# BiaPyX/BiaPy

Measured on AMD Instinct MI355X. Metric: voxels/sec 3D ResUNet 128^3 patch (train: fwd+bwd+AdamW; sub-records: infer, sliding), higher is better.
Workload: dtype f16 forward/activations + bf16 gradients (MFMA f16 / bf16, fp32 accumulate)

## Files before the change

### biapy_amd/_lib.py

```python
from __future__ import annotations

import ctypes as C
import os
from typing import Optional

import torch

_HERE = os.path.dirname(os.path.abspath(__file__))
LIB_PATH = os.environ.get("BPX_LIB_PATH") or os.path.join(_HERE, "libbiapy_amd.so")

F32, BF16, F16, U8, MIX16 = 0, 1, 2, 3, 4
U16 = 5
I32 = 6
ACT = {"none": 0, "linear": 0, "elu": 1, "relu": 2, "silu": 3, "leaky_relu": 4, "gelu": 5, "tanh": 6, "sigmoid": 7, "softplus": 8}
PK_K3, PK_K3_T, PK_K1, PK_DENSE, PK_DENSE_T, PK_CT, PK_CT_T, PK_CT4, PK_CT4_T = range(9)


class AxisGrid(C.Structure):
    _fields_ = [("n", C.c_int32), ("step", C.c_int32), ("last", C.c_int32), ("patch", C.c_int32), ("limit", C.c_int32)]


class Tensor(C.Structure):
    _fields_ = [("ptr", C.c_void_p), ("ld", C.c_int32), ("C", C.c_int32), ("cs", C.c_int64)]

# ... 95 lines not shown
    "bpx_conv3d_wgrad": ([_i, _i, _i, _i, _i, Tensor, _vp, _i, Tensor, _i, _vp, _vp, _vp, _i64, _vp], _i),
    "bpx_conv3d_wgrad_db2": ([_i, _i, _i, _i, _i, Tensor, _vp, _i, Tensor, _i, _vp, _vp, _vp, _vp, _i64, _vp], _i),
    "bpx_conv3d_wgrad_workspace": ([_i, _i, _i, _i, _i, _i, _i], _i64),
    "bpx_conv3d_bwd_fused_supported": ([_i, _i, _i, _i, _i, _i, _i], _i),
    "bpx_conv3d_bwd_fused_stats_tiles": ([_i, _i, _i, _i, _i, _i], _i),
    "bpx_conv3d_bwd_fused_workspace": ([_i, _i, _i, _i, _i, _i], _i64),
    "bpx_conv3d_bwd_fused": ([_i, _i, _i, _i, _i, Tensor, _vp, Tensor, _vp, _i, Tensor, _vp, _vp, _vp, _vp, _vp, _i64, _vp], _i),
    "bpx_debug_set_bwd_fused": ([_i], _i),
    "bpx_debug_set_bwd_rs": ([_i], _i),
    "bpx_debug_set_conv_kg": ([_i], _i),
    "bpx_debug_set_tile_order": ([_i], _i),
    "bpx_debug_set_wgrad_cap": ([_i], _i),
    "bpx_debug_set_wgrad_k1": ([_i], _i),
    "bpx_debug_set_pw_stream": ([_i], _i),
    "bpx_debug_set_convt_k1": ([_i], _i),
    "bpx_debug_set_c1_persist": ([_i], _i),
    "bpx_convT3d_k2s2_wgrad_workspace": ([_i, _i, _i, _i, _i, _i, _i], _i64),
    "bpx_conv1x1_fwd": ([_i, _i, _i64, Tensor, _vp, _vp, Tensor, Tensor, _vp, Tensor, Tensor, _vp], _i),
    "bpx_conv1x1_fwd_split_wgrad_workspace": ([_i, _i, _i64, _i], _i64),
    "bpx_conv1x1_fwd_split_wgrad_query": ([_i, _i, _i64, Tensor, Tensor, Tensor, _vp, Tensor, Tensor], _i64),
    "bpx_conv1x1_fwd_split_wgrad": ([_i, _i, _i64, Tensor, _vp, Tensor, Tensor, _vp, Tensor, Tensor, _vp, _vp, _i64, _vp], _i),
    "bpx_conv1x1_fwd_split": ([_i, _i, _i64, Tensor, _vp, _vp, Tensor, Tensor, _vp, Tensor, Tensor, Tensor, _vp], _i),
    "bpx_convT3d_k2s2_fwd": ([_i, _i, _i, _i, _i, _i, Tensor, _vp, _vp, Tensor, _vp, _vp], _i),
    "bpx_convT3d_stats_tiles": ([_i, _i, _i, _i], _i),
    "bpx_convT3d_k2s2_dgrad": ([_i, _i, _i, _i, _i, _i, Tensor, _vp, Tensor, _vp], _i),
    "bpx_convT3d_k2s2_wgrad": ([_i, _i, _i, _i, _i, _i, Tensor, Tensor, _vp, _vp, _vp, _i64, _vp], _i),
    "bpx_convT3d_k2s2_bwd": ([_i, _i, _i, _i, _i, _i, Tensor, Tensor, _vp, Tensor, _vp, _vp, _vp, _i64, _vp], _i),
    "bpx_debug_set_convt_bwd": ([_i], _i),
    "bpx_debug_convt_bwd_launches": ([], _i),
    "bpx_norm_finalize": ([_vp, _i, _i, _i, _i64, _vp, _vp, _f, _i, _vp, _i, _i, _vp], _i),
# ... 239 lines not shown
```

### biapy_amd/csrc/pointwise.hip

```cpp
#include <type_traits>

#include <cstdlib>

#include "bpx_common.h"

#ifndef BPX_PW_MS_CT
#define BPX_PW_MS_CT 2
#endif
#ifndef BPX_CONVT_OCC
#define BPX_CONVT_OCC 2
#endif
#ifndef BPX_CONVT_PD
#define BPX_CONVT_PD 2
#endif

namespace {

enum { PW_CONV1 = 0, PW_CONVT = 1, PW_CONVTD = 2 };

template <typename T> __device__ __forceinline__ void load4(const T* p, float* f);
template <> __device__ __forceinline__ void load4<uint16_t>(const uint16_t* p, float* f) {
  u32x2_t v = *reinterpret_cast<const u32x2_t*>(p);
  f[0] = bf16lo(v[0]); f[1] = bf16hi(v[0]); f[2] = bf16lo(v[1]); f[3] = bf16hi(v[1]);
}
template <> __device__ __forceinline__ void load4<float>(const float* p, float* f) {
  f32x4_t v = *reinterpret_cast<const f32x4_t*>(p);
  f[0] = v[0]; f[1] = v[1]; f[2] = v[2]; f[3] = v[3];
}

template <typename T, int NQ> __device__ __forceinline__ void loadq(const T* p, float (*f)[4]);
template <typename T, int NQ> __device__ __forceinline__ void storeq(T* p, const float (*f)[4]);
template <> __device__ __forceinline__ void loadq<float, 1>(const float* p, float (*f)[4]) { load4<float>(p, f[0]); }
template <> __device__ __forceinline__ void loadq<float, 2>(const float* p, float (*f)[4]) { load4<float>(p, f[0]); load4<float>(p + 4, f[1]); }
template <> __device__ __forceinline__ void loadq<float, 3>(const float* p, float (*f)[4]) { load4<float>(p, f[0]); load4<float>(p + 4, f[1]); load4<float>(p + 8, f[2]); }
template <> __device__ __forceinline__ void loadq<float, 4>(const float* p, float (*f)[4]) { load4<float>(p, f[0]); load4<float>(p + 4, f[1]); load4<float>(p + 8, f[2]); load4<float>(p + 12, f[3]); }
__device__ __forceinline__ void load8_bf16(const uint16_t* p, float* f0, float* f1) {
  u32x4_t v = *reinterpret_cast<const u32x4_t*>(p);
  f0[0] = bf16lo(v[0]); f0[1] = bf16hi(v[0]); f0[2] = bf16lo(v[1]); f0[3] = bf16hi(v[1]);
  f1[0] = bf16lo(v[2]); f1[1] = bf16hi(v[2]); f1[2] = bf16lo(v[3]); f1[3] = bf16hi(v[3]);
}
template <> __device__ __forceinline__ void loadq<uint16_t, 1>(const uint16_t* p, float (*f)[4]) { load4<uint16_t>(p, f[0]); }
template <> __device__ __forceinline__ void loadq<uint16_t, 2>(const uint16_t* p, float (*f)[4]) { load8_bf16(p, f[0], f[1]); }
template <> __device__ __forceinline__ void loadq<uint16_t, 3>(const uint16_t* p, float (*f)[4]) { load8_bf16(p, f[0], f[1]); load4<uint16_t>(p + 8, f[2]); }
template <> __device__ __forceinline__ void loadq<uint16_t, 4>(const uint16_t* p, float (*f)[4]) { load8_bf16(p, f[0], f[1]); load8_bf16(p + 8, f[2], f[3]); }
template <int NQ> __device__ __forceinline__ void storeq_f32(float* p, const float (*f)[4]) {
#pragma unroll
  for (int q = 0; q < NQ; ++q) *reinterpret_cast<f32x4_t*>(p + 4 * q) = f32x4_t{f[q][0], f[q][1], f[q][2], f[q][3]};
}
template <> __device__ __forceinline__ void storeq<float, 1>(float* p, const float (*f)[4]) { storeq_f32<1>(p, f); }
template <> __device__ __forceinline__ void storeq<float, 2>(float* p, const float (*f)[4]) { storeq_f32<2>(p, f); }
template <> __device__ __forceinline__ void storeq<float, 3>(float* p, const float (*f)[4]) { storeq_f32<3>(p, f); }
template <> __device__ __forceinline__ void storeq<float, 4>(float* p, const float (*f)[4]) { storeq_f32<4>(p, f); }
__device__ __forceinline__ void store4_bf16(uint16_t* p, const float* f) {
  *reinterpret_cast<u32x2_t*>(p) = u32x2_t{pack_bf16x2(f[0], f[1]), pack_bf16x2(f[2], f[3])};
}
__device__ __forceinline__ void store8_bf16(uint16_t* p, const float* f0, const float* f1) {
  *reinterpret_cast<u32x4_t*>(p) = u32x4_t{pack_bf16x2(f0[0], f0[1]), pack_bf16x2(f0[2], f0[3]), pack_bf16x2(f1[0], f1[1]), pack_bf16x2(f1[2], f1[3])};
}
template <> __device__ __forceinline__ void storeq<uint16_t, 1>(uint16_t* p, const float (*f)[4]) { store4_bf16(p, f[0]); }
template <> __device__ __forceinline__ void storeq<uint16_t, 2>(uint16_t* p, const float (*f)[4]) { store8_bf16(p, f[0], f[1]); }
template <> __device__ __forceinline__ void storeq<uint16_t, 3>(uint16_t* p, const float (*f)[4]) { store8_bf16(p, f[0], f[1]); store4_bf16(p + 8, f[2]); }
template <> __device__ __forceinline__ void storeq<uint16_t, 4>(uint16_t* p, const float (*f)[4]) { store8_bf16(p, f[0], f[1]); store8_bf16(p + 8, f[2], f[3]); }

template <> __device__ __forceinline__ void load4<f16_t>(const f16_t* p, float* f) {
  u32x2_t v = *reinterpret_cast<const u32x2_t*>(p);
  f[0] = lo16<f16_t>(v[0]); f[1] = hi16<f16_t>(v[0]); f[2] = lo16<f16_t>(v[1]); f[3] = hi16<f16_t>(v[1]);
}
__device__ __forceinline__ void load8_f16(const f16_t* p, float* f0, float* f1) {
  u32x4_t v = *reinterpret_cast<const u32x4_t*>(p);
  f0[0] = lo16<f16_t>(v[0]); f0[1] = hi16<f16_t>(v[0]); f0[2] = lo16<f16_t>(v[1]); f0[3] = hi16<f16_t>(v[1]);
  f1[0] = lo16<f16_t>(v[2]); f1[1] = hi16<f16_t>(v[2]); f1[2] = lo16<f16_t>(v[3]); f1[3] = hi16<f16_t>(v[3]);
}
template <> __device__ __forceinline__ void loadq<f16_t, 1>(const f16_t* p, float (*f)[4]) { load4<f16_t>(p, f[0]); }
template <> __device__ __forceinline__ void loadq<f16_t, 2>(const f16_t* p, float (*f)[4]) { load8_f16(p, f[0], f[1]); }
template <> __device__ __forceinline__ void loadq<f16_t, 3>(const f16_t* p, float (*f)[4]) { load8_f16(p, f[0], f[1]); load4<f16_t>(p + 8, f[2]); }
template <> __device__ __forceinline__ void loadq<f16_t, 4>(const f16_t* p, float (*f)[4]) { load8_f16(p, f[0], f[1]); load8_f16(p + 8, f[2], f[3]); }
__device__ __forceinline__ void store4_f16(f16_t* p, const float* f) {
  *reinterpret_cast<u32x2_t*>(p) = u32x2_t{pk16s<f16_t>(f[0], f[1]), pk16s<f16_t>(f[2], f[3])};
}
__device__ __forceinline__ void store8_f16(f16_t* p, const float* f0, const float* f1) {
  *reinterpret_cast<u32x4_t*>(p) = u32x4_t{pk16s<f16_t>(f0[0], f0[1]), pk16s<f16_t>(f0[2], f0[3]), pk16s<f16_t>(f1[0], f1[1]), pk16s<f16_t>(f1[2], f1[3])};
}
template <> __device__ __forceinline__ void storeq<f16_t, 1>(f16_t* p, const float (*f)[4]) { store4_f16(p, f[0]); }
template <> __device__ __forceinline__ void storeq<f16_t, 2>(f16_t* p, const float (*f)[4]) { store8_f16(p, f[0], f[1]); }
template <> __device__ __forceinline__ void storeq<f16_t, 3>(f16_t* p, const float (*f)[4]) { store8_f16(p, f[0], f[1]); store4_f16(p + 8, f[2]); }
template <> __device__ __forceinline__ void storeq<f16_t, 4>(f16_t* p, const float (*f)[4]) { store8_f16(p, f[0], f[1]); store8_f16(p + 8, f[2], f[3]); }

template <typename T, int NQ> __device__ __forceinline__ void loadq_planar(const T* vbase, int c0, int cs, float (*f)[4]) {
  auto at = [&](int c) { return vbase + (size_t)(c >> 4) * cs + (c & 15); };
  if (NQ == 1) loadq<T, 1>(at(c0), f);
  else if (NQ == 2) loadq<T, 2>(at(c0), f);
  else if (NQ == 4) { loadq<T, 2>(at(c0), f); loadq<T, 2>(at(c0 + 8), f + 2); }
  else if (sizeof(T) == 4) { loadq<T, 1>(at(c0), f); loadq<T, 1>(at(c0 + 4), f + 1); loadq<T, 1>(at(c0 + 8), f + 2); }
  else {
    const int b0 = c0 & ~7;
    float a[2][4], b[2][4];
    loadq<T, 2>(at(b0), a);
    loadq<T, 2>(at(b0 + 8), b);
    const bool odd = (c0 & 7) != 0;
#pragma unroll
    for (int r = 0; r < 4; ++r) {
      f[0][r] = odd ? a[1][r] : a[0][r];
      f[1][r] = odd ? b[0][r] : a[1][r];
      f[2][r] = odd ? b[1][r] : b[0][r];
    }
  }
}
template <typename T, int NQ> __device__ __forceinline__ void storeq_planar(T* vbase, int c0, int cs, const float (*f)[4]) {
  auto at = [&](int c) { return vbase + (size_t)(c >> 4) * cs + (c & 15); };
  if (NQ == 1) storeq<T, 1>(at(c0), f);
  else if (NQ == 2) storeq<T, 2>(at(c0), f);
  else if (NQ == 4) { storeq<T, 2>(at(c0), f); storeq<T, 2>(at(c0 + 8), f + 2); }
  else if ((c0 & 7) == 0) { storeq<T, 2>(at(c0), f); storeq<T, 1>(at(c0 + 8), f + 2); }
  else { storeq<T, 1>(at(c0), f); storeq<T, 2>(at(c0 + 4), f + 1); }
}

struct PwParams {
  int N, D, H, W;
  int sz;
  int64_t vps;
  const void* x; int x_ld; int K;
  int Csub;
  const void* wp; const float* bias;
  void* y; int y_ld; int Ncols;
  void* y2; int y2_ld; int ysplit;
  const void* g; int g_ld; const void* t; int t_ld; const bpx_nbwd_coef* coef;
  int t_cs, y_cs;
  const void* addend; int addend_ld;
  float* part; int mblocks;
  uint32_t y_bytes;
  int mgroups;
};

template <typename T, int MS, int NS, int MODE, bool PL, typename TT = T, bool K1STEP = false>
__global__ void __launch_bounds__(256) pw_kernel(const PwParams p) {
  using Tr = ElemTraits<T>;
  constexpr int KPL = Tr::KPL;
  const int tid = threadIdx.x, lane = tid & 63, wave = tid >> 6;
  const int j = lane & 15, g = lane >> 4;
  const int nbk = p.Ncols / (16 * NS);
  const unsigned bid = blockIdx.x;
  const int nb = bid % nbk;
  const int grp = (bid / nbk) % p.mgroups;
  const int n = bid / (nbk * p.mgroups);
  const int col_base = nb * 16 * NS;
  constexpr bool PERM = MODE == PW_CONVT && PL && NS == 4;
  const int ppb = PERM ? p.Csub / 32 : 1;
// ... 554 lines not shown
        }
      }
    __syncthreads();
    if (tid < NS * 16 * 2) {
      const int c = tid >> 1, k = tid & 1;
      const float a = red[(0 * NS * 16 + c) * 2 + k] + red[(1 * NS * 16 + c) * 2 + k] + red[(2 * NS * 16 + c) * 2 + k] + red[(3 * NS * 16 + c) * 2 + k];
      const int gg = c >> 4, ns = (c >> 2) & 3;
      const int sub_c = 2 * sp + (gg >> 1);
      const int co = pp * 32 + (ns >> 1) * 16 + (gg & 1) * 8 + (ns & 1) * 4 + (c & 3);
      p.part[((((size_t)n * p.mgroups + grp) * (4 * p.sz) + sub_c) * 2 + k) * p.Csub + co] = a;
    }
  }
}

int g_pw_stream = 1;
int g_convt_k1 = -1;
constexpr int PW_MS = 2;
constexpr int PW_MS_CT = BPX_PW_MS_CT;

inline int convt_groups(int64_t vps) { return (int)std::min<int64_t>(cdiv64(vps, 64 * PW_MS_CT), 64); }

inline int pw_ns(int ncols_per_group) { return (ncols_per_group % 64 == 0) ? 4 : (ncols_per_group % 48 == 0) ? 3 : (ncols_per_group % 32 == 0) ? 2 : 1; }

template <typename T, int MODE, typename TT = T>
int launch_pw(PwParams& p, int ns, hipStream_t s) {
  constexpr int MSK = (MODE == PW_CONVT) ? PW_MS_CT : PW_MS;
  if (p.vps >= (1ll << 31) - 64 * MSK) { bpx_set_error("pointwise kernels: more than 2^31 voxels per sample"); return 1; }
  p.mblocks = (int)cdiv64(p.vps, 64 * MSK);
  p.mgroups = MODE == PW_CONVT ? convt_groups(p.vps) : p.mblocks;
  int nbk = p.Ncols / (16 * ns);
  dim3 grid((unsigned)((int64_t)p.N * p.mgroups * nbk));
  const bool planar = (MODE == PW_CONV1 && p.coef != nullptr && p.t_cs != 16) || (MODE == PW_CONVT && p.y_cs != 16);
  if (MODE == PW_CONVT && planar && ns == 4 && p.Csub % 32 != 0) { bpx_set_error("transposed conv: the 64-column planar form needs Cout % 32 == 0"); return 1; }
  if (MODE != PW_CONVTD && planar) {
    constexpr bool PL = MODE != PW_CONVTD;
    if constexpr (MODE == PW_CONVT && sizeof(T) == 2) {
      const int64_t ovox = (int64_t)p.N * p.vps * 4 * p.sz;
      const int64_t ybytes = ((int64_t)(p.Csub / 16 - 1) * p.y_cs + (ovox - 1) * p.y_ld + 16) * 2;
      static const bool k1_env = getenv("BPX_CONVT_K1") == nullptr || atoi(getenv("BPX_CONVT_K1")) != 0;
      const bool k1 = g_convt_k1 < 0 ? k1_env : g_convt_k1 != 0;
      if (k1 && ns == 4 && p.K * 2 <= 64 && p.W % 16 == 0 && p.vps * p.x_ld * 2 < 0xFFFFFF00ll && ybytes < 0xFFFFFF00ll) {
        p.y_bytes = (uint32_t)ybytes;
        convt_k1_kernel<T><<<grid, 256, 0, s>>>(p);
        return 0;
      }
    }
    if (ns == 4 && MODE == PW_CONVT && sizeof(T) == 2 && p.K * (int)sizeof(T) <= 64) pw_kernel<T, MSK, 4, MODE, PL, TT, MODE == PW_CONVT && sizeof(T) == 2><<<grid, 256, 0, s>>>(p);
    else if (ns == 4) pw_kernel<T, MSK, 4, MODE, PL, TT><<<grid, 256, 0, s>>>(p);
// ... 9 lines not shown
  return 0;
}

int chk(const char* fn, const char* name, const bpx_tensor& t, int es) {
  BPX_CHECK(t.ptr != nullptr, "%s: %s.ptr is null", fn, name);
  BPX_CHECK(t.C % 16 == 0 && t.ld >= (t.cs ? 16 : t.C), "%s: %s needs C %% 16 == 0 and ld >= C (C=%d ld=%d)", fn, name, t.C, t.ld);
  BPX_CHECK(t.cs == 0 || t.cs % 8 == 0, "%s: %s has chunk stride %lld (must be a multiple of 8 elements)", fn, name, (long long)t.cs);
  BPX_CHECK(((uintptr_t)t.ptr % 16) == 0 && ((size_t)t.ld * es) % 16 == 0, "%s: %s must be 16-byte aligned", fn, name);
  return 0;
}

}

extern "C" int bpx_debug_set_pw_stream(int on) { g_pw_stream = on; return 0; }
extern "C" int bpx_debug_set_convt_k1(int on) { g_convt_k1 = on; return 0; }
extern "C" int bpx_convT3d_stats_tiles(int D, int H, int W, int sz) { return convt_groups((int64_t)D * H * W) * 4 * (sz == 1 ? 1 : 2); }

static bool pws_ok(int dtype, int N, int64_t vps, const bpx_tensor& x, bool has_coef, const float* bias_d, const bpx_tensor& g, const bpx_tensor& t,
                   const void* coef_d, const bpx_tensor& addend, const bpx_tensor& y, const bpx_tensor& y2) {
  const int KC = x.C / 16;
  const int TV = KC == 1 ? 128 : 64;
  const int64_t vox = (int64_t)N * vps;
  auto span = [&](const bpx_tensor& q, int chunks) { return (q.cs ? (int64_t)q.cs * (chunks - 1) : 0) * 2 + vox * (int64_t)q.ld * 2; };
  return g_pw_stream && dtype == BPX_BF16 && (KC == 1 || KC == 2) && x.C % 16 == 0 && has_coef && y2.ptr != nullptr && y.C + y2.C == 3 * x.C && y.C % 4 == 0 &&
         g.C == 3 * x.C && t.C == 3 * x.C && bias_d == nullptr && addend.ptr == nullptr && vps % TV == 0 && vox >= 262144 &&
         span(x, 1) < (1ll << 31) && span(g, 1) < (1ll << 31) && span(t, 3 * KC) < (1ll << 31) && (x.ld & 7) == 0 && (g.ld & 7) == 0 && (t.ld & 7) == 0 &&
         (y.ld & 3) == 0 && (y2.ld & 3) == 0 && (((uintptr_t)x.ptr | (uintptr_t)g.ptr | (uintptr_t)t.ptr | (uintptr_t)coef_d) & 15) == 0 &&
         (((uintptr_t)y.ptr | (uintptr_t)y2.ptr) & 7) == 0;
}

// ... 148 lines not shown
```

### include/biapy_amd.h

```cpp
#ifndef BIAPY_AMD_H
#define BIAPY_AMD_H

#include <stdint.h>

#ifdef __cplusplus
extern "C" {
#endif

typedef void* bpx_stream_t;

enum bpx_dtype { BPX_F32 = 0, BPX_BF16 = 1, BPX_F16 = 2, BPX_U8 = 3,
                 BPX_MIX16 = 4,
                 BPX_U16 = 5,
                 BPX_I32 = 6 };
enum bpx_act { BPX_ACT_NONE = 0, BPX_ACT_ELU = 1, BPX_ACT_RELU = 2, BPX_ACT_SILU = 3, BPX_ACT_LEAKY_RELU = 4, BPX_ACT_GELU = 5, BPX_ACT_TANH = 6,
               BPX_ACT_SIGMOID = 7, BPX_ACT_SOFTPLUS = 8, BPX_ACT_LAST = 8 };
enum bpx_pad_mode { BPX_PAD_REFLECT = 0, BPX_PAD_ZEROS = 1 };

int bpx_version(void);
const char* bpx_last_error(void);
int bpx_selftest_layouts(float* out_d , bpx_stream_t stream);
int bpx_debug_set_wgrad_tr(int use_tr);
int bpx_debug_set_conv_stamps(void* stamps_d);
int bpx_debug_set_conv_ws(int on);
int bpx_debug_set_conv_occ(int wg_per_cu);
int bpx_debug_set_conv_zm(int mode);
int bpx_debug_conv_zm_launches(void);
int bpx_debug_conv_zm_occupancy(int nch);
int bpx_debug_set_c1_persist(int wgs);
int bpx_debug_set_convt_k1(int on);
int bpx_debug_set_pw_stream(int on);
int bpx_debug_set_wgrad_k1(int on);
int bpx_debug_set_wgrad_cap(int percent);
int bpx_debug_set_tile_order(int bits);
int bpx_debug_set_tiling_scalar(int on);

typedef struct bpx_axis_grid {
  int32_t n, step, last, patch, limit;
} bpx_axis_grid;

int bpx_crop3d_gather(const void* vol_d, int elem_size, int Z, int Y, int X, int C,
                      int pad_z, int pad_y, int pad_x, int pad_mode,
                      const bpx_axis_grid* grid_zyx ,
                      int64_t c_begin, int64_t c_count, void* out_d, bpx_stream_t stream);

// ... 395 lines not shown
```

Baseline: 1.061 billion.

## Add software-pipelined pointwise GEMM kernel for transposed-conv dgrad path

Adds a separate pointwise kernel variant whose K loop keeps several weight and activation fragment loads in flight in register slots ahead of the MFMA steps. By default it is routed only to the transposed-conv dgrad mode, and only when K is large enough, with a bitmask so other modes can opt in. Shared helpers move into a common header. The intent is to hide global load latency in the K loop; the cost is higher register pressure, which could lower occupancy.

```diff
diff --git a/biapy_amd/_lib.py b/biapy_amd/_lib.py
--- a/biapy_amd/_lib.py
+++ b/biapy_amd/_lib.py
@@ -133,6 +133,7 @@
     "bpx_debug_set_wgrad_k1": ([_i], _i),
     "bpx_debug_set_pw_stream": ([_i], _i),
     "bpx_debug_set_convt_k1": ([_i], _i),
+    "bpx_debug_set_pw_pipeline": ([_i], _i),
     "bpx_debug_set_c1_persist": ([_i], _i),
     "bpx_convT3d_k2s2_wgrad_workspace": ([_i, _i, _i, _i, _i, _i, _i], _i64),
     "bpx_conv1x1_fwd": ([_i, _i, _i64, Tensor, _vp, _vp, Tensor, Tensor, _vp, Tensor, Tensor, _vp], _i),
diff --git a/biapy_amd/csrc/pointwise.hip b/biapy_amd/csrc/pointwise.hip
--- a/biapy_amd/csrc/pointwise.hip
+++ b/biapy_amd/csrc/pointwise.hip
@@ -14,123 +14,10 @@
 #define BPX_CONVT_PD 2
 #endif
 
+#include "pointwise_shared.h"
+
 namespace {
 
-enum { PW_CONV1 = 0, PW_CONVT = 1, PW_CONVTD = 2 };
-
-template <typename T> __device__ __forceinline__ void load4(const T* p, float* f);
-template <> __device__ __forceinline__ void load4<uint16_t>(const uint16_t* p, float* f) {
-  u32x2_t v = *reinterpret_cast<const u32x2_t*>(p);
-  f[0] = bf16lo(v[0]); f[1] = bf16hi(v[0]); f[2] = bf16lo(v[1]); f[3] = bf16hi(v[1]);
-}
-template <> __device__ __forceinline__ void load4<float>(const float* p, float* f) {
-  f32x4_t v = *reinterpret_cast<const f32x4_t*>(p);
-  f[0] = v[0]; f[1] = v[1]; f[2] = v[2]; f[3] = v[3];
-}
-
-template <typename T, int NQ> __device__ __forceinline__ void loadq(const T* p, float (*f)[4]);
-template <typename T, int NQ> __device__ __forceinline__ void storeq(T* p, const float (*f)[4]);
-template <> __device__ __forceinline__ void loadq<float, 1>(const float* p, float (*f)[4]) { load4<float>(p, f[0]); }
-template <> __device__ __forceinline__ void loadq<float, 2>(const float* p, float (*f)[4]) { load4<float>(p, f[0]); load4<float>(p + 4, f[1]); }
-template <> __device__ __forceinline__ void loadq<float, 3>(const float* p, float (*f)[4]) { load4<float>(p, f[0]); load4<float>(p + 4, f[1]); load4<float>(p + 8, f[2]); }
-template <> __device__ __forceinline__ void loadq<float, 4>(const float* p, float (*f)[4]) { load4<float>(p, f[0]); load4<float>(p + 4, f[1]); load4<float>(p + 8, f[2]); load4<float>(p + 12, f[3]); }
-__device__ __forceinline__ void load8_bf16(const uint16_t* p, float* f0, float* f1) {
-  u32x4_t v = *reinterpret_cast<const u32x4_t*>(p);
-  f0[0] = bf16lo(v[0]); f0[1] = bf16hi(v[0]); f0[2] = bf16lo(v[1]); f0[3] = bf16hi(v[1]);
-  f1[0] = bf16lo(v[2]); f1[1] = bf16hi(v[2]); f1[2] = bf16lo(v[3]); f1[3] = bf16hi(v[3]);
-}
-template <> __device__ __forceinline__ void loadq<uint16_t, 1>(const uint16_t* p, float (*f)[4]) { load4<uint16_t>(p, f[0]); }
-template <> __device__ __forceinline__ void loadq<uint16_t, 2>(const uint16_t* p, float (*f)[4]) { load8_bf16(p, f[0], f[1]); }
-template <> __device__ __forceinline__ void loadq<uint16_t, 3>(const uint16_t* p, float (*f)[4]) { load8_bf16(p, f[0], f[1]); load4<uint16_t>(p + 8, f[2]); }
-template <> __device__ __forceinline__ void loadq<uint16_t, 4>(const uint16_t* p, float (*f)[4]) { load8_bf16(p, f[0], f[1]); load8_bf16(p + 8, f[2], f[3]); }
-template <int NQ> __device__ __forceinline__ void storeq_f32(float* p, const float (*f)[4]) {
-#pragma unroll
-  for (int q = 0; q < NQ; ++q) *reinterpret_cast<f32x4_t*>(p + 4 * q) = f32x4_t{f[q][0], f[q][1], f[q][2], f[q][3]};
-}
-template <> __device__ __forceinline__ void storeq<float, 1>(float* p, const float (*f)[4]) { storeq_f32<1>(p, f); }
-template <> __device__ __forceinline__ void storeq<float, 2>(float* p, const float (*f)[4]) { storeq_f32<2>(p, f); }
-template <> __device__ __forceinline__ void storeq<float, 3>(float* p, const float (*f)[4]) { storeq_f32<3>(p, f); }
-template <> __device__ __forceinline__ void storeq<float, 4>(float* p, const float (*f)[4]) { storeq_f32<4>(p, f); }
-__device__ __forceinline__ void store4_bf16(uint16_t* p, const float* f) {
-  *reinterpret_cast<u32x2_t*>(p) = u32x2_t{pack_bf16x2(f[0], f[1]), pack_bf16x2(f[2], f[3])};
-}
-__device__ __forceinline__ void store8_bf16(uint16_t* p, const float* f0, const float* f1) {
-  *reinterpret_cast<u32x4_t*>(p) = u32x4_t{pack_bf16x2(f0[0], f0[1]), pack_bf16x2(f0[2], f0[3]), pack_bf16x2(f1[0], f1[1]), pack_bf16x2(f1[2], f1[3])};
-}
-template <> __device__ __forceinline__ void storeq<uint16_t, 1>(uint16_t* p, const float (*f)[4]) { store4_bf16(p, f[0]); }
-template <> __device__ __forceinline__ void storeq<uint16_t, 2>(uint16_t* p, const float (*f)[4]) { store8_bf16(p, f[0], f[1]); }
-template <> __device__ __forceinline__ void storeq<uint16_t, 3>(uint16_t* p, const float (*f)[4]) { store8_bf16(p, f[0], f[1]); store4_bf16(p + 8, f[2]); }
-template <> __device__ __forceinline__ void storeq<uint16_t, 4>(uint16_t* p, const float (*f)[4]) { store8_bf16(p, f[0], f[1]); store8_bf16(p + 8, f[2], f[3]); }
-
-template <> __device__ __forceinline__ void load4<f16_t>(const f16_t* p, float* f) {
-  u32x2_t v = *reinterpret_cast<const u32x2_t*>(p);
-  f[0] = lo16<f16_t>(v[0]); f[1] = hi16<f16_t>(v[0]); f[2] = lo16<f16_t>(v[1]); f[3] = hi16<f16_t>(v[1]);
-}
-__device__ __forceinline__ void load8_f16(const f16_t* p, float* f0, float* f1) {
-  u32x4_t v = *reinterpret_cast<const u32x4_t*>(p);
-  f0[0] = lo16<f16_t>(v[0]); f0[1] = hi16<f16_t>(v[0]); f0[2] = lo16<f16_t>(v[1]); f0[3] = hi16<f16_t>(v[1]);
-  f1[0] = lo16<f16_t>(v[2]); f1[1] = hi16<f16_t>(v[2]); f1[2] = lo16<f16_t>(v[3]); f1[3] = hi16<f16_t>(v[3]);
-}
-template <> __device__ __forceinline__ void loadq<f16_t, 1>(const f16_t* p, float (*f)[4]) { load4<f16_t>(p, f[0]); }
-template <> __device__ __forceinline__ void loadq<f16_t, 2>(const f16_t* p, float (*f)[4]) { load8_f16(p, f[0], f[1]); }
-template <> __device__ __forceinline__ void loadq<f16_t, 3>(const f16_t* p, float (*f)[4]) { load8_f16(p, f[0], f[1]); load4<f16_t>(p + 8, f[2]); }
-template <> __device__ __forceinline__ void loadq<f16_t, 4>(const f16_t* p, float (*f)[4]) { load8_f16(p, f[0], f[1]); load8_f16(p + 8, f[2], f[3]); }
-__device__ __forceinline__ void store4_f16(f16_t* p, const float* f) {
-  *reinterpret_cast<u32x2_t*>(p) = u32x2_t{pk16s<f16_t>(f[0], f[1]), pk16s<f16_t>(f[2], f[3])};
-}
-__device__ __forceinline__ void store8_f16(f16_t* p, const float* f0, const float* f1) {
-  *reinterpret_cast<u32x4_t*>(p) = u32x4_t{pk16s<f16_t>(f0[0], f0[1]), pk16s<f16_t>(f0[2], f0[3]), pk16s<f16_t>(f1[0], f1[1]), pk16s<f16_t>(f1[2], f1[3])};
-}
-template <> __device__ __forceinline__ void storeq<f16_t, 1>(f16_t* p, const float (*f)[4]) { store4_f16(p, f[0]); }
-template <> __device__ __forceinline__ void storeq<f16_t, 2>(f16_t* p, const float (*f)[4]) { store8_f16(p, f[0], f[1]); }
-template <> __device__ __forceinline__ void storeq<f16_t, 3>(f16_t* p, const float (*f)[4]) { store8_f16(p, f[0], f[1]); store4_f16(p + 8, f[2]); }
-template <> __device__ __forceinline__ void storeq<f16_t, 4>(f16_t* p, const float (*f)[4]) { store8_f16(p, f[0], f[1]); store8_f16(p + 8, f[2], f[3]); }
-
-template <typename T, int NQ> __device__ __forceinline__ void loadq_planar(const T* vbase, int c0, int cs, float (*f)[4]) {
-  auto at = [&](int c) { return vbase + (size_t)(c >> 4) * cs + (c & 15); };
-  if (NQ == 1) loadq<T, 1>(at(c0), f);
-  else if (NQ == 2) loadq<T, 2>(at(c0), f);
-  else if (NQ == 4) { loadq<T, 2>(at(c0), f); loadq<T, 2>(at(c0 + 8), f + 2); }
-  else if (sizeof(T) == 4) { loadq<T, 1>(at(c0), f); loadq<T, 1>(at(c0 + 4), f + 1); loadq<T, 1>(at(c0 + 8), f + 2); }
-  else {
-    const int b0 = c0 & ~7;
-    float a[2][4], b[2][4];
-    loadq<T, 2>(at(b0), a);
-    loadq<T, 2>(at(b0 + 8), b);
-    const bool odd = (c0 & 7) != 0;
-#pragma unroll
-    for (int r = 0; r < 4; ++r) {
-      f[0][r] = odd ? a[1][r] : a[0][r];
-      f[1][r] = odd ? b[0][r] : a[1][r];
-      f[2][r] = odd ? b[1][r] : b[0][r];
-    }
-  }
-}
-template <typename T, int NQ> __device__ __forceinline__ void storeq_planar(T* vbase, int c0, int cs, const float (*f)[4]) {
-  auto at = [&](int c) { return vbase + (size_t)(c >> 4) * cs + (c & 15); };
-  if (NQ == 1) storeq<T, 1>(at(c0), f);
-  else if (NQ == 2) storeq<T, 2>(at(c0), f);
-  else if (NQ == 4) { storeq<T, 2>(at(c0), f); storeq<T, 2>(at(c0 + 8), f + 2); }
-  else if ((c0 & 7) == 0) { storeq<T, 2>(at(c0), f); storeq<T, 1>(at(c0 + 8), f + 2); }
-  else { storeq<T, 1>(at(c0), f); storeq<T, 2>(at(c0 + 4), f + 1); }
-}
-
-struct PwParams {
-  int N, D, H, W;
-  int sz;
-  int64_t vps;
-  const void* x; int x_ld; int K;
-  int Csub;
-  const void* wp; const float* bias;
-  void* y; int y_ld; int Ncols;
-  void* y2; int y2_ld; int ysplit;
-  const void* g; int g_ld; const void* t; int t_ld; const bpx_nbwd_coef* coef;
-  int t_cs, y_cs;
-  const void* addend; int addend_ld;
-  float* part; int mblocks;
-  uint32_t y_bytes;
-  int mgroups;
-};
 
 template <typename T, int MS, int NS, int MODE, bool PL, typename TT = T, bool K1STEP = false>
 __global__ void __launch_bounds__(256) pw_kernel(const PwParams p) {
@@ -715,6 +602,8 @@
 }
 
 int g_pw_stream = 1;
+int g_pw_pipeline = -1;
+constexpr int PW_PIPE_DEFAULT = 8;
 int g_convt_k1 = -1;
 constexpr int PW_MS = 2;
 constexpr int PW_MS_CT = BPX_PW_MS_CT;
@@ -733,6 +622,15 @@
   dim3 grid((unsigned)((int64_t)p.N * p.mgroups * nbk));
   const bool planar = (MODE == PW_CONV1 && p.coef != nullptr && p.t_cs != 16) || (MODE == PW_CONVT && p.y_cs != 16);
   if (MODE == PW_CONVT && planar && ns == 4 && p.Csub % 32 != 0) { bpx_set_error("transposed conv: the 64-column planar form needs Cout % 32 == 0"); return 1; }
+  {
+    static const int pipe_env = getenv("BPX_PW_PIPELINE") == nullptr ? -1 : atoi(getenv("BPX_PW_PIPELINE"));
+    const int pipe_sel = g_pw_pipeline >= 0 ? g_pw_pipeline : pipe_env;
+    const int pipe_mask = pipe_sel < 0 ? PW_PIPE_DEFAULT : pipe_sel == 1 ? 14 : pipe_sel;
+    if (((pipe_mask >> (MODE + 1)) & 1) != 0 && p.K > 4 * ElemTraits<T>::KPL) {
+      const int r = bpx_pw_pipe_launch(MODE, ElemTraits<T>::DT, ElemTraits<TT>::DT, MSK, ns, planar ? 1 : 0, &p, grid.x, s);
+      if (r >= 0) return r;
+    }
+  }
   if (MODE != PW_CONVTD && planar) {
     constexpr bool PL = MODE != PW_CONVTD;
     if constexpr (MODE == PW_CONVT && sizeof(T) == 2) {
@@ -772,6 +670,7 @@
 
 extern "C" int bpx_debug_set_pw_stream(int on) { g_pw_stream = on; return 0; }
 extern "C" int bpx_debug_set_convt_k1(int on) { g_convt_k1 = on; return 0; }
+extern "C" int bpx_debug_set_pw_pipeline(int on) { g_pw_pipeline = on; return 0; }
 extern "C" int bpx_convT3d_stats_tiles(int D, int H, int W, int sz) { return convt_groups((int64_t)D * H * W) * 4 * (sz == 1 ? 1 : 2); }
 
 static bool pws_ok(int dtype, int N, int64_t vps, const bpx_tensor& x, bool has_coef, const float* bias_d, const bpx_tensor& g, const bpx_tensor& t,
diff --git a/biapy_amd/csrc/pointwise_pipe.hip b/biapy_amd/csrc/pointwise_pipe.hip
--- /dev/null
+++ b/biapy_amd/csrc/pointwise_pipe.hip
@@ -0,0 +1,374 @@
+#include "pointwise_shared.h"
+
+#define BPX_CONVT_PD 1
+
+namespace {
+
+template <int I, int N, typename F> __device__ __forceinline__ void pw_static_for(F&& f) {
+  if constexpr (I < N) { f(std::integral_constant<int, I>{}); pw_static_for<I + 1, N>(f); }
+}
+template <typename T, int MS, int NS, int MODE, bool PL, typename TT, bool K1STEP, int PIPE>
+__device__ __forceinline__ void pw_body(const PwParams& p) {
+  using Tr = ElemTraits<T>;
+  constexpr int KPL = Tr::KPL;
+  const int tid = threadIdx.x, lane = tid & 63, wave = tid >> 6;
+  const int j = lane & 15, g = lane >> 4;
+  const int nbk = p.Ncols / (16 * NS);
+  const unsigned bid = blockIdx.x;
+  const int nb = bid % nbk;
+  const int grp = (bid / nbk) % p.mgroups;
+  const int n = bid / (nbk * p.mgroups);
+  const int col_base = nb * 16 * NS;
+  constexpr bool PERM = MODE == PW_CONVT && PL && NS == 4;
+  const int ppb = PERM ? p.Csub / 32 : 1;
+  const int sp = nb / ppb, pp = nb - sp * ppb;
+
+  float s1[NS][4], s2[NS][4];
+#pragma unroll
+  for (int ns = 0; ns < NS; ++ns)
+#pragma unroll
+    for (int r = 0; r < 4; ++r) s1[ns][r] = s2[ns][r] = 0.f;
+  T* __restrict__ yout = reinterpret_cast<T*>(p.y);
+  const T* __restrict__ xin = reinterpret_cast<const T*>(p.x);
+  const T* __restrict__ wp = reinterpret_cast<const T*>(p.wp);
+
+  int mb = grp;
+  constexpr bool PRE = MODE == PW_CONVT && K1STEP;
+  constexpr bool pre = PRE;
+  constexpr int PD = PRE ? BPX_CONVT_PD : 1;
+  u32x4_t af_pre[PD][PRE ? MS : 1], wf_keep[PRE ? NS : 1];
+  auto prefetch = [&](int mbn, auto slot_c) {
+    constexpr int SL = decltype(slot_c)::value;
+#pragma unroll
+    for (int ms = 0; ms < (PRE ? MS : 1); ++ms) {
+      const uint32_t vn = ((uint32_t)mbn * 4u + (uint32_t)wave) * (uint32_t)(MS * 16) + (uint32_t)(ms * 16 + j);
+      af_pre[SL][ms] = u32x4_t{0u, 0u, 0u, 0u};
+      if (g * KPL < p.K && vn < (uint32_t)p.vps) af_pre[SL][ms] = *reinterpret_cast<const u32x4_t*>(xin + ((size_t)n * p.vps + vn) * (size_t)p.x_ld + g * KPL);
+    }
+  };
+  if (pre) {
+    prefetch(mb, std::integral_constant<int, 0>{});
+    if (PD > 1 && mb + p.mgroups < p.mblocks) prefetch(mb + p.mgroups, std::integral_constant<int, (PD > 1 ? 1 : 0)>{});
+    if (PD > 2 && mb + 2 * p.mgroups < p.mblocks) prefetch(mb + 2 * p.mgroups, std::integral_constant<int, (PD > 2 ? 2 : 0)>{});
+    if (PD > 3 && mb + 3 * p.mgroups < p.mblocks) prefetch(mb + 3 * p.mgroups, std::integral_constant<int, (PD > 3 ? 3 : 0)>{});
+#pragma unroll
+    for (int ns = 0; ns < (PRE ? NS : 1); ++ns) {
+      const int gq = j >> 2;
+      const int colw = PERM ? (2 * sp + (gq >> 1)) * p.Csub + pp * 32 + (ns >> 1) * 16 + (gq & 1) * 8 + (ns & 1) * 4 + (j & 3)
+                            : col_base + gq * (4 * NS) + ns * 4 + (j & 3);
+      wf_keep[ns] = *reinterpret_cast<const u32x4_t*>(wp + ((size_t)g * p.Ncols + colw) * KPL);
+    }
+  }
+  const int col0 = col_base + g * 4 * NS;
+  int sub = 0, co0 = col0;
+  if (MODE == PW_CONVT) { sub = col0 / p.Csub; co0 = col0 % p.Csub; }
+  if (PERM) { sub = 2 * sp + (g >> 1); co0 = pp * 32 + (g & 1) * 8; }
+  auto cof = [&](int ns) { return PERM ? co0 + (ns >> 1) * 16 + (ns & 1) * 4 : co0 + ns * 4; };
+  float add[NS][4];
+  auto load_bias = [&]() {
+#pragma unroll
+    for (int ns = 0; ns < NS; ++ns)
+#pragma unroll
+      for (int r = 0; r < 4; ++r) add[ns][r] = p.bias ? p.bias[cof(ns) + r] : 0.f;
+  };
+  if (MODE == PW_CONVT) load_bias();
+  auto one_block = [&](auto slot_c) {
+  constexpr int SL = decltype(slot_c)::value;
+  uint32_t v[MS];
+  bool valid[MS];
+  size_t abase[MS];
+  uint32_t cx[MS], cy[MS], cz[MS];
+#pragma unroll
+  for (int ms = 0; ms < MS; ++ms) {
+    v[ms] = ((uint32_t)mb * 4u + (uint32_t)wave) * (uint32_t)(MS * 16) + (uint32_t)(ms * 16 + j);
+    valid[ms] = v[ms] < (uint32_t)p.vps;
+    const uint32_t vv = valid[ms] ? v[ms] : 0u;
+    if (MODE != PW_CONV1) {
+      const uint32_t row = vv / (uint32_t)p.W;
+      cx[ms] = vv - row * (uint32_t)p.W;
+      cz[ms] = row / (uint32_t)p.H;
+      cy[ms] = row - cz[ms] * (uint32_t)p.H;
+    }
+    if (MODE == PW_CONVTD) {
+      abase[ms] = ((((size_t)n * p.sz * p.D + p.sz * cz[ms]) * 2 * p.H + 2 * cy[ms]) * 2 * p.W + 2 * cx[ms]) * (size_t)p.x_ld;
+    } else {
+      abase[ms] = ((size_t)n * p.vps + vv) * (size_t)p.x_ld;
+    }
+  }
+
+  f32x4_t acc[MS][NS];
+#pragma unroll
+  for (int ms = 0; ms < MS; ++ms)
+#pragma unroll
+    for (int ns = 0; ns < NS; ++ns) acc[ms][ns] = f32x4_t{0.f, 0.f, 0.f, 0.f};
+
+  const int ksteps = (p.K / KPL + 3) / 4;
+  auto plain_loop = [&]() {
+  for (int s = 0; s < ksteps; ++s) {
+    const int k = (4 * s + g) * KPL;
+    const bool kin = k < p.K;
+    u32x4_t wf[NS];
+#pragma unroll
+    for (int ns = 0; ns < NS; ++ns)
+    {
+      if (PRE && pre) { wf[ns] = wf_keep[PRE ? ns : 0]; continue; }
+      const int gq = j >> 2;
+      const int colw = PERM ? (2 * sp + (gq >> 1)) * p.Csub + pp * 32 + (ns >> 1) * 16 + (gq & 1) * 8 + (ns & 1) * 4 + (j & 3)
+                            : col_base + gq * (4 * NS) + ns * 4 + (j & 3);
+      wf[ns] = *reinterpret_cast<const u32x4_t*>(wp + ((size_t)(4 * s + g) * p.Ncols + colw) * KPL);
+    }
+    size_t koff;
+    if (MODE == PW_CONVTD) {
+      int sub = kin ? k / p.Csub : 0, c = kin ? k % p.Csub : 0;
+      int a = (sub >> 2) & 1, b = (sub >> 1) & 1, cc = sub & 1;
+      koff = (((size_t)a * 2 * p.H + b) * 2 * p.W + cc) * (size_t)p.x_ld + c;
+    } else {
+      koff = kin ? k : 0;
+    }
+#pragma unroll
+    for (int ms = 0; ms < MS; ++ms) {
+      u32x4_t af = u32x4_t{0u, 0u, 0u, 0u};
+      if (PRE && pre) af = af_pre[SL][PRE ? ms : 0];
+      else if (kin && valid[ms]) af = *reinterpret_cast<const u32x4_t*>(xin + abase[ms] + koff);
+#pragma unroll
+      for (int ns = 0; ns < NS; ++ns) acc[ms][ns] = mfma_step<T>(wf[ns], af, acc[ms][ns]);
+    }
+  }
+  };
+  if constexpr (PIPE == 0) {
+    plain_loop();
+  } else if (ksteps < PIPE) {
+    plain_loop();
+  } else {
+    constexpr int R = PIPE, NSL = R + 1;
+    u32x4_t wfr[NSL][NS], afr[NSL][MS];
+    const int gq = j >> 2;
+    const T* wreq = wp + ((size_t)g * p.Ncols + (PERM ? (2 * sp + (gq >> 1)) * p.Csub + pp * 32 + (gq & 1) * 8 + (j & 3) : col_base + gq * (4 * NS) + (j & 3))) * KPL;
+    const size_t wstep = (size_t)4 * p.Ncols * KPL;
+    int rk = g * KPL;
+    int rsub = 0, rc = rk;
+    if (MODE == PW_CONVTD) { rsub = rk >= p.Csub ? 1 : 0; rc = rk - rsub * p.Csub; }
+    auto request = [&](auto slot_c) {
+      constexpr int SLT = decltype(slot_c)::value;
+#pragma unroll
+      for (int ns = 0; ns < NS; ++ns) wfr[SLT][ns] = *reinterpret_cast<const u32x4_t*>(wreq + (PERM ? (ns >> 1) * 16 + (ns & 1) * 4 : ns * 4) * KPL);
+      wreq += wstep;
+      size_t koff;
+      if (MODE == PW_CONVTD) {
+        const bool kin = rsub < 4 * p.sz;
+        const int sb = kin ? rsub : 0, c = kin ? rc : 0;
+        const int a = (sb >> 2) & 1, b = (sb >> 1) & 1, cc = sb & 1;
+        koff = (((size_t)a * 2 * p.H + b) * 2 * p.W + cc) * (size_t)p.x_ld + c;
+        rc += 4 * KPL;
+        if (rc >= p.Csub) { rc -= p.Csub; ++rsub; }
+        if (rc >= p.Csub) { rc -= p.Csub; ++rsub; }
+      } else {
+        koff = rk < p.K ? rk : 0;
+      }
+      rk += 4 * KPL;
+#pragma unroll
+      for (int ms = 0; ms < MS; ++ms) afr[SLT][ms] = *reinterpret_cast<const u32x4_t*>(xin + abase[ms] + koff);
+    };
+    auto consume = [&](auto slot_c, int s) {
+      constexpr int SLT = decltype(slot_c)::value;
+      const bool kin = (4 * s + g) * KPL < p.K;
+#pragma unroll
+      for (int ms = 0; ms < MS; ++ms) {
+        u32x4_t af = afr[SLT][ms];
+        if (!(kin && valid[ms])) af = u32x4_t{0u, 0u, 0u, 0u};
+#pragma unroll
+        for (int ns = 0; ns < NS; ++ns) acc[ms][ns] = mfma_step<T>(wfr[SLT][ns], af, acc[ms][ns]);
+      }
+    };
+    pw_static_for<0, R>([&](auto r) { request(r); });
+    int s = 0;
+    while (s + NSL - 1 + R < ksteps) {
+      pw_static_for<0, NSL>([&](auto u) {
+        request(std::integral_constant<int, (decltype(u)::value + R) % NSL>{});
+        __builtin_amdgcn_sched_barrier(0);
+        consume(u, s);
+        ++s;
+        __builtin_amdgcn_sched_barrier(0);
+      });
+    }
+    auto tail = [&](auto self, auto u) -> void {
+      constexpr int U = decltype(u)::value;
+      if constexpr (U < NSL - 1) {
+        if (s + R < ksteps) {
+          request(std::integral_constant<int, (U + R) % NSL>{});
+          __builtin_amdgcn_sched_barrier(0);
+          consume(u, s);
+          ++s;
+          self(self, std::integral_constant<int, U + 1>{});
+          return;
+        }
+      }
+      pw_static_for<0, R>([&](auto i) { consume(std::integral_constant<int, (U + decltype(i)::value) % NSL>{}, s + decltype(i)::value); });
+    };
+    tail(tail, std::integral_constant<int, 0>{});
+    static_assert(R >= 2 && R <= 4, "ring depth");
+  }
+  if (PRE && pre && mb + PD * p.mgroups < p.mblocks) prefetch(mb + PD * p.mgroups, slot_c);
+
+  if (MODE != PW_CONVT) load_bias();
+  bpx_nbwd_coef cf[NS][4];
+  if (MODE == PW_CONV1 && p.coef) {
+#pragma unroll
+    for (int ns = 0; ns < NS; ++ns)
+#pragma unroll
+      for (int r = 0; r < 4; ++r) cf[ns][r] = p.coef[(size_t)n * p.Ncols + co0 + ns * 4 + r];
+  }
+#pragma unroll
+  for (int ms = 0; ms < MS; ++ms) {
+    if (!valid[ms]) continue;
+    size_t ovox;
+    if (MODE == PW_CONVT) {
+      const int xw = (int)cx[ms], yh = (int)cy[ms], zd = (int)cz[ms];
+      int a = (sub >> 2) & 1, b = (sub >> 1) & 1, cc = sub & 1;
+      ovox = (((size_t)n * p.sz * p.D + p.sz * zd + a) * 2 * p.H + 2 * yh + b) * 2 * p.W + 2 * xw + cc;
+    } else {
+      ovox = (size_t)n * p.vps + v[ms];
+    }
+    float val[NS][4];
+#pragma unroll
+    for (int ns = 0; ns < NS; ++ns)
+#pragma unroll
+      for (int r = 0; r < 4; ++r) val[ns][r] = acc[ms][ns][r] + add[ns][r];
+    if (MODE == PW_CONV1) {
+      if (p.coef) {
+        float gq[NS][4], tq[NS][4];
+        loadq<T, NS>(reinterpret_cast<const T*>(p.g) + ovox * (size_t)p.g_ld + co0, gq);
+        if (!PL) loadq<TT, NS>(reinterpret_cast<const TT*>(p.t) + ovox * (size_t)p.t_ld + co0, tq);
+        else loadq_planar<TT, NS>(reinterpret_cast<const TT*>(p.t) + ovox * (size_t)p.t_ld, co0, p.t_cs, tq);
+#pragma unroll
+        for (int ns = 0; ns < NS; ++ns)
+#pragma unroll
+          for (int r = 0; r < 4; ++r) val[ns][r] += cf[ns][r].a * gq[ns][r] + cf[ns][r].b * tq[ns][r] + cf[ns][r].c0;
+      }
+      if (p.addend) {
+        float aq[NS][4];
+        loadq<T, NS>(reinterpret_cast<const T*>(p.addend) + ovox * (size_t)p.addend_ld + co0, aq);
+#pragma unroll
+        for (int ns = 0; ns < NS; ++ns)
+#pragma unroll
+          for (int r = 0; r < 4; ++r) val[ns][r] += aq[ns][r];
+      }
+    }
+    if (MODE == PW_CONVT) {
+#pragma unroll
+      for (int ns = 0; ns < NS; ++ns)
+#pragma unroll
+        for (int r = 0; r < 4; ++r) { s1[ns][r] += val[ns][r]; s2[ns][r] += val[ns][r] * val[ns][r]; }
+    }
+    if (MODE == PW_CONV1 && p.y2 != nullptr) {
+#pragma unroll
+      for (int ns = 0; ns < NS; ++ns) {
+        const int col = co0 + ns * 4;
+        T* dst = col < p.ysplit ? yout + ovox * (size_t)p.y_ld + col : reinterpret_cast<T*>(p.y2) + ovox * (size_t)p.y2_ld + (col - p.ysplit);
+        storeq<T, 1>(dst, val + ns);
+      }
+    } else if (!PL) {
+      storeq<T, NS>(yout + ovox * (size_t)p.y_ld + co0, val);
+    } else if (PERM) {
+      T* vb = yout + ovox * (size_t)p.y_ld;
+      storeq<T, 2>(vb + (size_t)(co0 >> 4) * p.y_cs + (co0 & 15), val);
+      storeq<T, 2>(vb + (size_t)((co0 >> 4) + 1) * p.y_cs + (co0 & 15), val + (NS > 2 ? 2 : 0));
+    } else {
+      storeq_planar<T, NS>(yout + ovox * (size_t)p.y_ld, co0, p.y_cs, val);
+    }
+  }
+
+  };
+  if constexpr (PD == 1) {
+    do { one_block(std::integral_constant<int, 0>{}); } while (MODE == PW_CONVT && (mb += p.mgroups) < p.mblocks);
+  } else {
+    for (;;) {
+      one_block(std::integral_constant<int, 0>{});
+      if ((mb += p.mgroups) >= p.mblocks) break;
+      one_block(std::integral_constant<int, 1>{});
+      if ((mb += p.mgroups) >= p.mblocks) break;
+      if constexpr (PD > 2) {
+        one_block(std::integral_constant<int, (PD > 2 ? 2 : 0)>{});
+        if ((mb += p.mgroups) >= p.mblocks) break;
+      }
+      if constexpr (PD > 3) {
+        one_block(std::integral_constant<int, (PD > 3 ? 3 : 0)>{});
+        if ((mb += p.mgroups) >= p.mblocks) break;
+      }
+    }
+  }
+
+  mb = grp;
+  if (MODE == PW_CONVT && p.part != nullptr) {
+    __shared__ float red[4 * NS * 16 * 2];
+#pragma unroll
+    for (int ns = 0; ns < NS; ++ns)
+#pragma unroll
+      for (int r = 0; r < 4; ++r) {
+        const float a = row16_sum(s1[ns][r]), b = row16_sum(s2[ns][r]);
+        if (j == 0) {
+          red[((wave * NS * 16) + g * 4 * NS + ns * 4 + r) * 2 + 0] = a;
+          red[((wave * NS * 16) + g * 4 * NS + ns * 4 + r) * 2 + 1] = b;
+        }
+      }
+    __syncthreads();
+    if (tid < NS * 16 * 2) {
+      int c = tid >> 1, k = tid & 1;
+      float a = red[(0 * NS * 16 + c) * 2 + k] + red[(1 * NS * 16 + c) * 2 + k] + red[(2 * NS * 16 + c) * 2 + k] +
+                red[(3 * NS * 16 + c) * 2 + k];
+      int col = col_base + c, sub = col / p.Csub, co = col % p.Csub;
+      if (PERM) {
+        const int gg = c >> 4, ns = (c >> 2) & 3;
+        sub = 2 * sp + (gg >> 1);
+        co = pp * 32 + (ns >> 1) * 16 + (gg & 1) * 8 + (ns & 1) * 4 + (c & 3);
+      }
+      p.part[((((size_t)n * p.mgroups + mb) * (4 * p.sz) + sub) * 2 + k) * p.Csub + co] = a;
+    }
+  }
+}
+
+template <int MODE> constexpr int pw_ring() { return MODE == PW_CONVTD ? 4 : 2; }
+template <typename T, int MS, int NS, int MODE, bool PL, typename TT = T>
+__global__ void __launch_bounds__(256) pw_pipe_kernel(const PwParams p) { pw_body<T, MS, NS, MODE, PL, TT, false, pw_ring<MODE>()>(p); }
+
+
+
+template <typename T, int MODE, typename TT>
+int launch(const PwParams& p, int ns, bool planar, unsigned grid, hipStream_t s) {
+  if constexpr (MODE != PW_CONVTD) {
+    if (planar) {
+      if (ns == 4) pw_pipe_kernel<T, 2, 4, MODE, true, TT><<<grid, 256, 0, s>>>(p);
+      else if (ns == 3) pw_pipe_kernel<T, 2, 3, MODE, true, TT><<<grid, 256, 0, s>>>(p);
+      else if (ns == 2) pw_pipe_kernel<T, 2, 2, MODE, true, TT><<<grid, 256, 0, s>>>(p);
+      else pw_pipe_kernel<T, 2, 1, MODE, true, TT><<<grid, 256, 0, s>>>(p);
+      return 0;
+    }
+  }
+  if (ns == 4) pw_pipe_kernel<T, 2, 4, MODE, false, TT><<<grid, 256, 0, s>>>(p);
+  else if (ns == 3) pw_pipe_kernel<T, 2, 3, MODE, false, TT><<<grid, 256, 0, s>>>(p);
+  else if (ns == 2) pw_pipe_kernel<T, 2, 2, MODE, false, TT><<<grid, 256, 0, s>>>(p);
+  else pw_pipe_kernel<T, 2, 1, MODE, false, TT><<<grid, 256, 0, s>>>(p);
+  return 0;
+}
+
+}
+
+int bpx_pw_pipe_launch(int mode, int dt, int tt, int ms, int ns, int planar, const void* params, unsigned grid, hipStream_t s) {
+  const PwParams& p = *static_cast<const PwParams*>(params);
+  if (ms != 2 || ns < 1 || ns > 4) return -1;
+  const bool pl = planar != 0;
+  if (mode == PW_CONV1) {
+    if (dt == BPX_BF16 && tt == BPX_F16) return launch<uint16_t, PW_CONV1, f16_t>(p, ns, pl, grid, s);
+    if (dt == BPX_BF16 && tt == BPX_BF16) return launch<uint16_t, PW_CONV1, uint16_t>(p, ns, pl, grid, s);
+    if (dt == BPX_F16 && tt == BPX_F16) return launch<f16_t, PW_CONV1, f16_t>(p, ns, pl, grid, s);
+    if (dt == BPX_F32 && tt == BPX_F32) return launch<float, PW_CONV1, float>(p, ns, pl, grid, s);
+  } else if (mode == PW_CONVT && dt == tt) {
+    if (dt == BPX_BF16) return launch<uint16_t, PW_CONVT, uint16_t>(p, ns, pl, grid, s);
+    if (dt == BPX_F16) return launch<f16_t, PW_CONVT, f16_t>(p, ns, pl, grid, s);
+    if (dt == BPX_F32) return launch<float, PW_CONVT, float>(p, ns, pl, grid, s);
+  } else if (mode == PW_CONVTD && dt == tt && !pl) {
+    if (dt == BPX_BF16) return launch<uint16_t, PW_CONVTD, uint16_t>(p, ns, false, grid, s);
+    if (dt == BPX_F32) return launch<float, PW_CONVTD, float>(p, ns, false, grid, s);
+  }
+  return -1;
+}
diff --git a/biapy_amd/csrc/pointwise_shared.h b/biapy_amd/csrc/pointwise_shared.h
--- /dev/null
+++ b/biapy_amd/csrc/pointwise_shared.h
@@ -0,0 +1,128 @@
+#pragma once
+#include <type_traits>
+
+#include <cstdlib>
+
+#include "bpx_common.h"
+
+namespace {
+
+enum { PW_CONV1 = 0, PW_CONVT = 1, PW_CONVTD = 2 };
+
+template <typename T> __device__ __forceinline__ void load4(const T* p, float* f);
+template <> __device__ __forceinline__ void load4<uint16_t>(const uint16_t* p, float* f) {
+  u32x2_t v = *reinterpret_cast<const u32x2_t*>(p);
+  f[0] = bf16lo(v[0]); f[1] = bf16hi(v[0]); f[2] = bf16lo(v[1]); f[3] = bf16hi(v[1]);
+}
+template <> __device__ __forceinline__ void load4<float>(const float* p, float* f) {
+  f32x4_t v = *reinterpret_cast<const f32x4_t*>(p);
+  f[0] = v[0]; f[1] = v[1]; f[2] = v[2]; f[3] = v[3];
+}
+
+template <typename T, int NQ> __device__ __forceinline__ void loadq(const T* p, float (*f)[4]);
+template <typename T, int NQ> __device__ __forceinline__ void storeq(T* p, const float (*f)[4]);
+template <> __device__ __forceinline__ void loadq<float, 1>(const float* p, float (*f)[4]) { load4<float>(p, f[0]); }
+template <> __device__ __forceinline__ void loadq<float, 2>(const float* p, float (*f)[4]) { load4<float>(p, f[0]); load4<float>(p + 4, f[1]); }
+template <> __device__ __forceinline__ void loadq<float, 3>(const float* p, float (*f)[4]) { load4<float>(p, f[0]); load4<float>(p + 4, f[1]); load4<float>(p + 8, f[2]); }
+template <> __device__ __forceinline__ void loadq<float, 4>(const float* p, float (*f)[4]) { load4<float>(p, f[0]); load4<float>(p + 4, f[1]); load4<float>(p + 8, f[2]); load4<float>(p + 12, f[3]); }
+__device__ __forceinline__ void load8_bf16(const uint16_t* p, float* f0, float* f1) {
+  u32x4_t v = *reinterpret_cast<const u32x4_t*>(p);
+  f0[0] = bf16lo(v[0]); f0[1] = bf16hi(v[0]); f0[2] = bf16lo(v[1]); f0[3] = bf16hi(v[1]);
+  f1[0] = bf16lo(v[2]); f1[1] = bf16hi(v[2]); f1[2] = bf16lo(v[3]); f1[3] = bf16hi(v[3]);
+}
+template <> __device__ __forceinline__ void loadq<uint16_t, 1>(const uint16_t* p, float (*f)[4]) { load4<uint16_t>(p, f[0]); }
+template <> __device__ __forceinline__ void loadq<uint16_t, 2>(const uint16_t* p, float (*f)[4]) { load8_bf16(p, f[0], f[1]); }
+template <> __device__ __forceinline__ void loadq<uint16_t, 3>(const uint16_t* p, float (*f)[4]) { load8_bf16(p, f[0], f[1]); load4<uint16_t>(p + 8, f[2]); }
+template <> __device__ __forceinline__ void loadq<uint16_t, 4>(const uint16_t* p, float (*f)[4]) { load8_bf16(p, f[0], f[1]); load8_bf16(p + 8, f[2], f[3]); }
+template <int NQ> __device__ __forceinline__ void storeq_f32(float* p, const float (*f)[4]) {
+#pragma unroll
+  for (int q = 0; q < NQ; ++q) *reinterpret_cast<f32x4_t*>(p + 4 * q) = f32x4_t{f[q][0], f[q][1], f[q][2], f[q][3]};
+}
+template <> __device__ __forceinline__ void storeq<float, 1>(float* p, const float (*f)[4]) { storeq_f32<1>(p, f); }
+template <> __device__ __forceinline__ void storeq<float, 2>(float* p, const float (*f)[4]) { storeq_f32<2>(p, f); }
+template <> __device__ __forceinline__ void storeq<float, 3>(float* p, const float (*f)[4]) { storeq_f32<3>(p, f); }
+template <> __device__ __forceinline__ void storeq<float, 4>(float* p, const float (*f)[4]) { storeq_f32<4>(p, f); }
+__device__ __forceinline__ void store4_bf16(uint16_t* p, const float* f) {
+  *reinterpret_cast<u32x2_t*>(p) = u32x2_t{pack_bf16x2(f[0], f[1]), pack_bf16x2(f[2], f[3])};
+}
+__device__ __forceinline__ void store8_bf16(uint16_t* p, const float* f0, const float* f1) {
+  *reinterpret_cast<u32x4_t*>(p) = u32x4_t{pack_bf16x2(f0[0], f0[1]), pack_bf16x2(f0[2], f0[3]), pack_bf16x2(f1[0], f1[1]), pack_bf16x2(f1[2], f1[3])};
+}
+template <> __device__ __forceinline__ void storeq<uint16_t, 1>(uint16_t* p, const float (*f)[4]) { store4_bf16(p, f[0]); }
+template <> __device__ __forceinline__ void storeq<uint16_t, 2>(uint16_t* p, const float (*f)[4]) { store8_bf16(p, f[0], f[1]); }
+template <> __device__ __forceinline__ void storeq<uint16_t, 3>(uint16_t* p, const float (*f)[4]) { store8_bf16(p, f[0], f[1]); store4_bf16(p + 8, f[2]); }
+template <> __device__ __forceinline__ void storeq<uint16_t, 4>(uint16_t* p, const float (*f)[4]) { store8_bf16(p, f[0], f[1]); store8_bf16(p + 8, f[2], f[3]); }
+
+template <> __device__ __forceinline__ void load4<f16_t>(const f16_t* p, float* f) {
+  u32x2_t v = *reinterpret_cast<const u32x2_t*>(p);
+  f[0] = lo16<f16_t>(v[0]); f[1] = hi16<f16_t>(v[0]); f[2] = lo16<f16_t>(v[1]); f[3] = hi16<f16_t>(v[1]);
+}
+__device__ __forceinline__ void load8_f16(const f16_t* p, float* f0, float* f1) {
+  u32x4_t v = *reinterpret_cast<const u32x4_t*>(p);
+  f0[0] = lo16<f16_t>(v[0]); f0[1] = hi16<f16_t>(v[0]); f0[2] = lo16<f16_t>(v[1]); f0[3] = hi16<f16_t>(v[1]);
+  f1[0] = lo16<f16_t>(v[2]); f1[1] = hi16<f16_t>(v[2]); f1[2] = lo16<f16_t>(v[3]); f1[3] = hi16<f16_t>(v[3]);
+}
+template <> __device__ __forceinline__ void loadq<f16_t, 1>(const f16_t* p, float (*f)[4]) { load4<f16_t>(p, f[0]); }
+template <> __device__ __forceinline__ void loadq<f16_t, 2>(const f16_t* p, float (*f)[4]) { load8_f16(p, f[0], f[1]); }
+template <> __device__ __forceinline__ void loadq<f16_t, 3>(const f16_t* p, float (*f)[4]) { load8_f16(p, f[0], f[1]); load4<f16_t>(p + 8, f[2]); }
+template <> __device__ __forceinline__ void loadq<f16_t, 4>(const f16_t* p, float (*f)[4]) { load8_f16(p, f[0], f[1]); load8_f16(p + 8, f[2], f[3]); }
+__device__ __forceinline__ void store4_f16(f16_t* p, const float* f) {
+  *reinterpret_cast<u32x2_t*>(p) = u32x2_t{pk16s<f16_t>(f[0], f[1]), pk16s<f16_t>(f[2], f[3])};
+}
+__device__ __forceinline__ void store8_f16(f16_t* p, const float* f0, const float* f1) {
+  *reinterpret_cast<u32x4_t*>(p) = u32x4_t{pk16s<f16_t>(f0[0], f0[1]), pk16s<f16_t>(f0[2], f0[3]), pk16s<f16_t>(f1[0], f1[1]), pk16s<f16_t>(f1[2], f1[3])};
+}
+template <> __device__ __forceinline__ void storeq<f16_t, 1>(f16_t* p, const float (*f)[4]) { store4_f16(p, f[0]); }
+template <> __device__ __forceinline__ void storeq<f16_t, 2>(f16_t* p, const float (*f)[4]) { store8_f16(p, f[0], f[1]); }
+template <> __device__ __forceinline__ void storeq<f16_t, 3>(f16_t* p, const float (*f)[4]) { store8_f16(p, f[0], f[1]); store4_f16(p + 8, f[2]); }
+template <> __device__ __forceinline__ void storeq<f16_t, 4>(f16_t* p, const float (*f)[4]) { store8_f16(p, f[0], f[1]); store8_f16(p + 8, f[2], f[3]); }
+
+template <typename T, int NQ> __device__ __forceinline__ void loadq_planar(const T* vbase, int c0, int cs, float (*f)[4]) {
+  auto at = [&](int c) { return vbase + (size_t)(c >> 4) * cs + (c & 15); };
+  if (NQ == 1) loadq<T, 1>(at(c0), f);
+  else if (NQ == 2) loadq<T, 2>(at(c0), f);
+  else if (NQ == 4) { loadq<T, 2>(at(c0), f); loadq<T, 2>(at(c0 + 8), f + 2); }
+  else if (sizeof(T) == 4) { loadq<T, 1>(at(c0), f); loadq<T, 1>(at(c0 + 4), f + 1); loadq<T, 1>(at(c0 + 8), f + 2); }
+  else {
+    const int b0 = c0 & ~7;
+    float a[2][4], b[2][4];
+    loadq<T, 2>(at(b0), a);
+    loadq<T, 2>(at(b0 + 8), b);
+    const bool odd = (c0 & 7) != 0;
+#pragma unroll
+    for (int r = 0; r < 4; ++r) {
+      f[0][r] = odd ? a[1][r] : a[0][r];
+      f[1][r] = odd ? b[0][r] : a[1][r];
+      f[2][r] = odd ? b[1][r] : b[0][r];
+    }
+  }
+}
+template <typename T, int NQ> __device__ __forceinline__ void storeq_planar(T* vbase, int c0, int cs, const float (*f)[4]) {
+  auto at = [&](int c) { return vbase + (size_t)(c >> 4) * cs + (c & 15); };
+  if (NQ == 1) storeq<T, 1>(at(c0), f);
+  else if (NQ == 2) storeq<T, 2>(at(c0), f);
+  else if (NQ == 4) { storeq<T, 2>(at(c0), f); storeq<T, 2>(at(c0 + 8), f + 2); }
+  else if ((c0 & 7) == 0) { storeq<T, 2>(at(c0), f); storeq<T, 1>(at(c0 + 8), f + 2); }
+  else { storeq<T, 1>(at(c0), f); storeq<T, 2>(at(c0 + 4), f + 1); }
+}
+
+struct PwParams {
+  int N, D, H, W;
+  int sz;
+  int64_t vps;
+  const void* x; int x_ld; int K;
+  int Csub;
+  const void* wp; const float* bias;
+  void* y; int y_ld; int Ncols;
+  void* y2; int y2_ld; int ysplit;
+  const void* g; int g_ld; const void* t; int t_ld; const bpx_nbwd_coef* coef;
+  int t_cs, y_cs;
+  const void* addend; int addend_ld;
+  float* part; int mblocks;
+  uint32_t y_bytes;
+  int mgroups;
+};
+
+}
+
+int bpx_pw_pipe_launch(int mode, int dt, int tt, int ms, int ns, int planar, const void* params, unsigned grid, hipStream_t stream);
diff --git a/include/biapy_amd.h b/include/biapy_amd.h
--- a/include/biapy_amd.h
+++ b/include/biapy_amd.h
@@ -29,6 +29,7 @@
 int bpx_debug_conv_zm_occupancy(int nch);
 int bpx_debug_set_c1_persist(int wgs);
 int bpx_debug_set_convt_k1(int on);
+int bpx_debug_set_pw_pipeline(int on);
 int bpx_debug_set_pw_stream(int on);
 int bpx_debug_set_wgrad_k1(int on);
 int bpx_debug_set_wgrad_cap(int percent);
```

Measured after the change: 1.058 billion. Within noise of the previous version (-0.3%).
